# zju3dv/disprcnn

Hardware: AMD Instinct MI355X
Metric: ROI cost-volumes/sec (112x112x48) (higher is better)
Workload: dtype f32 (every convolution of the regressor, the three 32->1 heads included: split-f16 -- each fp32 value carried as hi + lo fp16, 3 f16-MFMA products per fp32 product, f32 accumulate; fp32-class error, tests/test_hip_s16.py.  Head gather and soft-argmin: f32 VALU); 1 GPU; Config A: per ROI pair, features [32,28,28]x2 -> concat cost volume [64,12,28,28] (folded into the first 3D layer's loads, never written) -> 3D stacked-hourglass regressor -> trilinear x4 + softmax + soft-argmin -> disparity [112,112]; maxdisp=48, mindisp=0, parallelism=roi-shard x1 (no collective), weights=closed-form synthetic (disprcnn_amd.utils.synth), BN stats calibrated fixture

## Files before the change

### disprcnn_amd/csrc/s16_cvrows.h

```cpp
#pragma once
#include <hip/hip_runtime.h>
#include <stdint.h>

#include "../../include/disprcnn_hip.h"
#include "s16_ovf.h"

namespace s16cv {

typedef float f32x4 __attribute__((ext_vector_type(4)));
typedef float f32x16 __attribute__((ext_vector_type(16)));
typedef unsigned u32x4 __attribute__((ext_vector_type(4)));
typedef _Float16 f16x8 __attribute__((ext_vector_type(8)));

constexpr int TX = 28;
constexpr int PG = 32;
constexpr int STG_TILE = 8 * 3 * 32 * 16;
constexpr int MAP_B = 32 * 128;
constexpr int MAP_TILE = 9 * MAP_B;
constexpr int STG0 = 0, MAPS0 = 3 * STG_TILE, ZCOL0 = MAPS0 + 3 * MAP_TILE;
constexpr int LDS_BYTES = ZCOL0 + 128;
static_assert(LDS_BYTES <= 160 * 1024, "LDS");

#define S16CV_LDS_PTR(p) ((__attribute__((address_space(3))) void*)(p))
#define S16CV_WAITCNT(vm, lgkm) (((vm) & 15) | (7 << 4) | ((lgkm) << 8) | (((vm) >> 4) << 14))

struct Task { unsigned n; int y, x0, j0, j1; bool valid; };

template <int ROWS>
__device__ __forceinline__ void s16_cvrows_run(const drc_s16conv_params& p, char* lds) {
    const int wave = __builtin_amdgcn_readfirstlane(threadIdx.x >> 6);
    const int lane = threadIdx.x & 63;
    const int xl = lane & 31, hf = lane >> 5;
    const int n_ct = p.cout / 32;
    const int ct = (int)((blockIdx.x >> 3) % n_ct);
    const int D = p.D, H = p.H, W = p.W, lo4 = p.lo4;
    const int Wp = W + 2, Hp = H + 2;
    const long rowB = (long)Wp * 128;
    const long planeB = (long)Hp * rowB;
    const long xcbB = (long)(D + 2) * planeB;
    const long ynB = (long)n_ct * xcbB;
    const long mapnB = planeB;

    const int side = wave >> 1, mlo = (wave & 1) * 4;
    f16x8 wh[5][3][2], wl[5][3][2];
#pragma unroll
    for (int mi = 0; mi < 5; ++mi) {
        const int m = mlo + mi, kd = m / 3, kw = m - kd * 3;
#pragma unroll
        for (int kh = 0; kh < 3; ++kh)
#pragma unroll
            for (int s = 0; s < 2; ++s) {
                const int t = kd * 9 + kh * 3 + kw;
                const char* wb = (const char*)p.w + ((long)(ct * 4 + side * 2 + s) * 54 + t * 2) * 1024 + lane * 16;
                wh[mi][kh][s] = *(const f16x8*)wb;
                wl[mi][kh][s] = *(const f16x8*)(wb + 1024);
            }
    }
    constexpr int PIN_WH = 14;
#pragma unroll
    for (int mi = 0; mi < 5; ++mi)
#pragma unroll
        for (int kh = 0; kh < 3; ++kh)
#pragma unroll
            for (int s = 0; s < 2; ++s) {
                asm volatile("" : "+a"(wl[mi][kh][s]));
                if ((mi * 3 + kh) * 2 + s < PIN_WH) asm volatile("" : "+a"(wh[mi][kh][s]));
            }
    const int q8 = wave * 2 + hf, sg = q8 & 3, jpar = wave >> 1;
    const int grp0 = (sg >> 1) * 4 + (sg & 1), grp1 = grp0 + 2;
    float sc[8], sh[8];
#pragma unroll
    for (int e = 0; e < 8; ++e) {
        const int co = ct * 32 + (sg >> 1) * 16 + (sg & 1) * 4 + 8 * (e >> 2) + (e & 3);
        sc[e] = p.scale[co];
        sh[e] = p.shift[co];
    }
    const float relu_lo = p.relu ? 0.f : -65504.f;
    const unsigned lo_off = (unsigned)(4 * Wp * 16);
    int s_chunk[3], s_row[3], s_col[3];
#pragma unroll
    for (int i = 0; i < 3; ++i) {
        const int idx = (wave * 3 + i) * 64 + lane;
        s_chunk[i] = idx / 96;
        const int rem = idx - s_chunk[i] * 96;
        s_row[i] = rem >> 5;
        s_col[i] = rem & 31;
    }
    if (threadIdx.x < 8) *(f32x4*)(lds + ZCOL0 + threadIdx.x * 16) = (f32x4){0.f, 0.f, 0.f, 0.f};

    const int n_xt = (W + TX - 1) / TX, n_yt = (H + ROWS - 1) / ROWS, n_pg = (D + PG - 1) / PG;
    const unsigned xcd = blockIdx.x & 7, qx = (blockIdx.x >> 3) / n_ct, per_xcd = (gridDim.x >> 3) / n_ct;
    const unsigned items_unit = (unsigned)n_yt * n_xt * n_pg;
    auto task_of = [&](unsigned idx) __attribute__((always_inline)) {
        Task t;
        for (;; ++idx) {
            const unsigned it = idx / ROWS, rr = idx - it * ROWS;
            const unsigned j = it * per_xcd + qx;
            const unsigned nl = j / items_unit;
            unsigned rem = j - nl * items_unit;
            const int yb = (int)(rem / (unsigned)(n_xt * n_pg));
            rem -= (unsigned)yb * (n_xt * n_pg);
            const int xt = (int)(rem / (unsigned)n_pg), pg = (int)(rem - (unsigned)xt * n_pg);
            t.n = nl * 8 + xcd;
            t.valid = t.n < (unsigned)p.N;
            t.y = yb * ROWS + (int)rr;
            t.x0 = xt * TX;
            t.j0 = pg * PG;
            t.j1 = t.j0 + PG < D ? t.j0 + PG : D;
            if (!t.valid || t.y < H) break;
        }
        struct R { Task t; unsigned idx; } r = {t, idx};
        return r;
    };
    struct Reach { int vlo, nb; };
    auto reach_of = [&](const Task& t) __attribute__((always_inline)) {
        Reach r;
        int vlo = t.x0 - (lo4 + t.j1 - 1) - 2, vhi = t.x0 + TX + 1 - (lo4 + t.j0);
        vlo = vlo > 0 ? vlo : 0;
        vhi = vhi < W - 1 ? vhi : W - 1;
        r.vlo = vlo;
        r.nb = vhi >= vlo ? ((vhi - vlo) >> 5) + 1 : 0;
        return r;
    };
    auto stage = [&](const Task& t) __attribute__((always_inline)) {
        const Reach rc = reach_of(t);
        const __amdgpu_buffer_rsrc_t ra = __builtin_amdgcn_make_buffer_rsrc((void*)((const char*)p.left + (long)t.n * mapnB), 0, 0x7FFFFF00, 0x00020000);
        const __amdgpu_buffer_rsrc_t rb = __builtin_amdgcn_make_buffer_rsrc((void*)((const char*)p.right + (long)t.n * mapnB), 0, 0x7FFFFF00, 0x00020000);
#pragma unroll
        for (int T = 0; T < 3; ++T) {
            if (T > rc.nb) break;
            const int v0 = T == 0 ? t.x0 - 1 : rc.vlo + (T - 1) * 32;
#pragma unroll
            for (int i = 0; i < 3; ++i) {
                const int v = v0 + s_col[i];
                const bool ok = v >= -1 && v <= W;
                const unsigned off = ok ? (unsigned)((long)(t.y + s_row[i]) * rowB + (long)s_chunk[i] * (Wp * 16) + (long)(v + 1) * 16) : 0u;
                char* dst = lds + STG0 + T * STG_TILE + (wave * 3 + i) * 1024;
                if (T == 0) __builtin_amdgcn_raw_ptr_buffer_load_lds(ra, S16CV_LDS_PTR(dst), 16, off, 0, 0, 0);
                else __builtin_amdgcn_raw_ptr_buffer_load_lds(rb, S16CV_LDS_PTR(dst), 16, off, 0, 0, 0);
            }
        }
    };
    typedef const __attribute__((address_space(3))) f16x8 lds_frag;
    typedef const __attribute__((address_space(3))) f32x4 lds_f4;
    const __attribute__((address_space(3))) char* ldsl = (const __attribute__((address_space(3))) char*)lds;

    auto cur = task_of(0);
    if (!cur.t.valid) return;
    S16Ovf og;
#pragma unroll
    for (int e = 0; e < 8; ++e) { og.see_raw(sc[e], 3.0e38f); og.see_raw(sh[e], 3.0e38f); }
    stage(cur.t);
#pragma unroll 1
    for (;;) {
        const Task t = cur.t;
        const Reach rc = reach_of(t);
        asm volatile("" ::: "memory");
        __builtin_amdgcn_s_waitcnt(S16CV_WAITCNT(0, 0));
        __builtin_amdgcn_s_barrier();
        asm volatile("" ::: "memory");
        const int nt = side ? rc.nb : 1;
#pragma unroll 1
        for (int T = 0; T < nt; ++T) {
            const int tile = side + T;
            const unsigned fb = (unsigned)(STG0 + tile * STG_TILE + (hf * 96 + xl) * 16);
            f32x16 acc[5];
#pragma unroll
            for (int mi = 0; mi < 5; ++mi)
#pragma unroll
                for (int e = 0; e < 16; ++e) acc[mi][e] = 0.f;
#pragma unroll
            for (int kh = 0; kh < 3; ++kh)
#pragma unroll
                for (int s = 0; s < 2; ++s) {
                    const f16x8 bh = *(lds_frag*)(ldsl + fb + (s * 2 * 96 + kh * 32) * 16);
                    const f16x8 bl = *(lds_frag*)(ldsl + fb + ((4 + s * 2) * 96 + kh * 32) * 16);
#pragma unroll
                    for (int mi = 0; mi < 5; ++mi) acc[mi] = __builtin_amdgcn_mfma_f32_32x32x16_f16(wh[mi][kh][s], bh, acc[mi], 0, 0, 0);
#pragma unroll
                    for (int mi = 0; mi < 5; ++mi) acc[mi] = __builtin_amdgcn_mfma_f32_32x32x16_f16(wh[mi][kh][s], bl, acc[mi], 0, 0, 0);
#pragma unroll
                    for (int mi = 0; mi < 5; ++mi) acc[mi] = __builtin_amdgcn_mfma_f32_32x32x16_f16(wl[mi][kh][s], bh, acc[mi], 0, 0, 0);
                }
#pragma unroll
            for (int mi = 0; mi < 5; ++mi) {
                if (mi == 0 && mlo != 0) continue;
                char* mb = lds + MAPS0 + tile * MAP_TILE + (mlo + mi) * MAP_B + xl * 128;
#pragma unroll
                for (int q = 0; q < 4; ++q)
                    *(f32x4*)(mb + (((2 * q + hf) ^ (xl & 7)) * 16)) = (f32x4){acc[mi][q * 4], acc[mi][q * 4 + 1], acc[mi][q * 4 + 2], acc[mi][q * 4 + 3]};
            }
        }
        asm volatile("" ::: "memory");
        __builtin_amdgcn_s_waitcnt(S16CV_WAITCNT(63, 0));
        __builtin_amdgcn_s_barrier();
        asm volatile("" ::: "memory");
        const auto nxt = task_of(cur.idx + 1);
        if (nxt.t.valid) stage(nxt.t);
        const int x = t.x0 + xl;
        const bool lane_ok = xl < TX && x < W;
        const unsigned long long og_keep = S16Ovf::lanes(lane_ok);
        const __amdgpu_buffer_rsrc_t y16r = __builtin_amdgcn_make_buffer_rsrc((char*)p.y16 + (long)t.n * ynB, 0, 0x7FFFFF00, 0x00020000);
        const unsigned o16 = (unsigned)((long)ct * xcbB + planeB + (long)(t.y + 1) * rowB + (long)sg * (Wp * 16) + (long)(x + 1) * 16);
        const int xa0 = t.x0 - 1;
#pragma unroll 1
        for (int j = t.j0 + jpar; j < t.j1; j += 2) {
            const int u = x - (lo4 + j);
            f32x4 a0 = {0.f, 0.f, 0.f, 0.f}, a1 = {0.f, 0.f, 0.f, 0.f};
#pragma unroll
            for (int kd = 0; kd < 3; ++kd) {
                const bool kd_ok = lane_ok && j + kd - 1 >= 0 && j + kd - 1 < D;
#pragma unroll
                for (int kw = 0; kw < 3; ++kw) {
                    const int cA = x + kw - 1, cB = u + kw - kd;
                    const bool ok = kd_ok && cA >= 0 && cA < W && cB >= 0 && cB < W;
                    const int ia = cA - xa0, ib = cB - rc.vlo;
                    const int m = kd * 3 + kw;
                    const unsigned colA = ok ? (unsigned)(MAPS0 + m * MAP_B + ia * 128) : (unsigned)ZCOL0;
                    const unsigned colB = ok ? (unsigned)(MAPS0 + MAP_TILE + (ib >> 5) * MAP_TILE + m * MAP_B + (ib & 31) * 128) : (unsigned)ZCOL0;
                    const unsigned swA = (unsigned)(ia & 7), swB = (unsigned)(ib & 7);
                    const f32x4 A0 = *(lds_f4*)(ldsl + colA + ((grp0 ^ swA) * 16)), A1 = *(lds_f4*)(ldsl + colA + ((grp1 ^ swA) * 16));
                    const f32x4 B0 = *(lds_f4*)(ldsl + colB + ((grp0 ^ swB) * 16)), B1 = *(lds_f4*)(ldsl + colB + ((grp1 ^ swB) * 16));
                    a0 += A0 + B0;
                    a1 += A1 + B1;
                }
            }
            f16x8 hi, lo;
#pragma unroll
            for (int e = 0; e < 8; ++e) {
                const float s_ = e < 4 ? a0[e & 3] : a1[e & 3];
                float x_ = s_ * sc[e] + sh[e];
                x_ = __builtin_amdgcn_fmed3f(x_, relu_lo, 65504.f);
                og.see(x_, og_keep);
                hi[e] = (_Float16)x_;
                lo[e] = (_Float16)(x_ - (float)hi[e]);
            }
            const unsigned po = lane_ok ? (unsigned)((long)j * planeB) : 0x80000000u;
            __builtin_amdgcn_raw_buffer_store_b128(__builtin_bit_cast(u32x4, hi), y16r, o16 + po, 0, 0);
            __builtin_amdgcn_raw_buffer_store_b128(__builtin_bit_cast(u32x4, lo), y16r, o16 + lo_off + po, 0, 0);
        }
        if (!nxt.t.valid) break;
        cur = nxt;
    }
    og.flush(p.ovf);
}

template <int ROWS>
inline long s16_cvrows_blocks(const drc_s16conv_params& p) {
    const long items = (long)p.N * ((p.H + ROWS - 1) / ROWS) * ((p.W + TX - 1) / TX) * ((p.D + PG - 1) / PG);
    const int n_ct = p.cout / 32;
    long blocks = 256;
    while (blocks > 8 * n_ct && blocks / (2 * n_ct) >= items) blocks /= 2;
    return blocks;
}

}
```

Baseline: 60450 ROI cost-volumes/s.

## Hoist j-invariant A-side map reads out of the disparity loop and rotate B offsets

The A-side map values (left-feature contributions) do not depend on disparity j, so they are now loaded once per task into registers instead of every j iteration. This halves the LDS reads in the inner loop. B-side column offsets are carried in a sliding window of five and shifted by two per step rather than recomputed. The loop also uses a mask-FMA in place of the zero-column trick for A, and adds explicit waitcnt and sched_barrier per kd to interleave reads and adds. The cost is 72 extra VGPRs for the A values, which may lower occupancy, and the forced scheduling may serialise LDS latency.

After: 61440 ROI cost-volumes/s, median of 6. 1.6% higher.

```diff
diff --git a/disprcnn_amd/csrc/s16_cvrows.h b/disprcnn_amd/csrc/s16_cvrows.h
--- a/disprcnn_amd/csrc/s16_cvrows.h
+++ b/disprcnn_amd/csrc/s16_cvrows.h
@@ -20,6 +20,7 @@
 constexpr int STG0 = 0, MAPS0 = 3 * STG_TILE, ZCOL0 = MAPS0 + 3 * MAP_TILE;
 constexpr int LDS_BYTES = ZCOL0 + 128;
 static_assert(LDS_BYTES <= 160 * 1024, "LDS");
+static_assert(ZCOL0 % 64 == 0, "a column's second cout group is its first ^ 32, in the zero column too");
 
 #define S16CV_LDS_PTR(p) ((__attribute__((address_space(3))) void*)(p))
 #define S16CV_WAITCNT(vm, lgkm) (((vm) & 15) | (7 << 4) | ((lgkm) << 8) | (((vm) >> 4) << 14))
@@ -67,7 +68,7 @@
                 if ((mi * 3 + kh) * 2 + s < PIN_WH) asm volatile("" : "+a"(wh[mi][kh][s]));
             }
     const int q8 = wave * 2 + hf, sg = q8 & 3, jpar = wave >> 1;
-    const int grp0 = (sg >> 1) * 4 + (sg & 1), grp1 = grp0 + 2;
+    const int grp0 = (sg >> 1) * 4 + (sg & 1);
     float sc[8], sh[8];
 #pragma unroll
     for (int e = 0; e < 8; ++e) {
@@ -202,28 +203,75 @@
         const unsigned long long og_keep = S16Ovf::lanes(lane_ok);
         const __amdgpu_buffer_rsrc_t y16r = __builtin_amdgcn_make_buffer_rsrc((char*)p.y16 + (long)t.n * ynB, 0, 0x7FFFFF00, 0x00020000);
         const unsigned o16 = (unsigned)((long)ct * xcbB + planeB + (long)(t.y + 1) * rowB + (long)sg * (Wp * 16) + (long)(x + 1) * 16);
-        const int xa0 = t.x0 - 1;
+        auto col_off = [&](unsigned c) __attribute__((always_inline)) { return c * 128u + (((unsigned)grp0 ^ (c & 7u)) << 4); };
+        bool okA[3];
+        f32x4 ar0[9], ar1[9];
+#pragma unroll
+        for (int kw = 0; kw < 3; ++kw) {
+            const int cA = x + kw - 1;
+            okA[kw] = lane_ok && cA >= 0 && cA < W;
+        }
+#pragma unroll
+        for (int m = 0; m < 9; ++m) {
+            const int kw = m % 3;
+            const unsigned oa = okA[kw] ? (unsigned)MAPS0 + col_off((unsigned)(xl + kw) & 31u) : (unsigned)(ZCOL0 - m * MAP_B);
+            ar0[m] = *(lds_f4*)(ldsl + oa + m * MAP_B);
+            ar1[m] = *(lds_f4*)(ldsl + (oa ^ 32u) + m * MAP_B);
+        }
+        auto off_of = [&](int cB) __attribute__((always_inline)) {
+            const int ib = cB - rc.vlo;
+            return (unsigned)(MAPS0 + MAP_TILE) + (unsigned)(ib >> 5) * (unsigned)MAP_TILE + col_off((unsigned)ib & 31u);
+        };
+        unsigned offB[5];
+        bool okB[5];
+        const int jb = t.j0 + jpar;
+#pragma unroll
+        for (int d = 0; d < 5; ++d) {
+            const int cB = x - (lo4 + jb) + d - 2;
+            offB[d] = off_of(cB);
+            okB[d] = (unsigned)cB < (unsigned)W;
+        }
 #pragma unroll 1
-        for (int j = t.j0 + jpar; j < t.j1; j += 2) {
-            const int u = x - (lo4 + j);
+        for (int j = jb; j < t.j1; j += 2) {
             f32x4 a0 = {0.f, 0.f, 0.f, 0.f}, a1 = {0.f, 0.f, 0.f, 0.f};
+            f32x4 B0[9], B1[9];
+            float msk[9];
+            auto read = [&](int kd) __attribute__((always_inline)) {
+                const bool kd_ok = j + kd - 1 >= 0 && j + kd - 1 < D;
+#pragma unroll
+                for (int kw = 0; kw < 3; ++kw) {
+                    const int m = kd * 3 + kw, d = kw - kd + 2;
+                    const bool ok = okA[kw] && kd_ok && okB[d];
+                    const unsigned ob = ok ? offB[d] : (unsigned)(ZCOL0 - m * MAP_B);
+                    B0[m] = *(lds_f4*)(ldsl + ob + m * MAP_B);
+                    B1[m] = *(lds_f4*)(ldsl + (ob ^ 32u) + m * MAP_B);
+                    msk[m] = ok ? 1.f : 0.f;
+                }
+            };
+            auto add = [&](int kd) __attribute__((always_inline)) {
+#pragma unroll
+                for (int kw = 0; kw < 3; ++kw) {
+                    const int m = kd * 3 + kw;
+                    const f32x4 k = {msk[m], msk[m], msk[m], msk[m]};
+                    a0 += __builtin_elementwise_fma(ar0[m], k, B0[m]);
+                    a1 += __builtin_elementwise_fma(ar1[m], k, B1[m]);
+                }
+            };
 #pragma unroll
             for (int kd = 0; kd < 3; ++kd) {
-                const bool kd_ok = lane_ok && j + kd - 1 >= 0 && j + kd - 1 < D;
-#pragma unroll
-                for (int kw = 0; kw < 3; ++kw) {
-                    const int cA = x + kw - 1, cB = u + kw - kd;
-                    const bool ok = kd_ok && cA >= 0 && cA < W && cB >= 0 && cB < W;
-                    const int ia = cA - xa0, ib = cB - rc.vlo;
-                    const int m = kd * 3 + kw;
-                    const unsigned colA = ok ? (unsigned)(MAPS0 + m * MAP_B + ia * 128) : (unsigned)ZCOL0;
-                    const unsigned colB = ok ? (unsigned)(MAPS0 + MAP_TILE + (ib >> 5) * MAP_TILE + m * MAP_B + (ib & 31) * 128) : (unsigned)ZCOL0;
-                    const unsigned swA = (unsigned)(ia & 7), swB = (unsigned)(ib & 7);
-                    const f32x4 A0 = *(lds_f4*)(ldsl + colA + ((grp0 ^ swA) * 16)), A1 = *(lds_f4*)(ldsl + colA + ((grp1 ^ swA) * 16));
-                    const f32x4 B0 = *(lds_f4*)(ldsl + colB + ((grp0 ^ swB) * 16)), B1 = *(lds_f4*)(ldsl + colB + ((grp1 ^ swB) * 16));
-                    a0 += A0 + B0;
-                    a1 += A1 + B1;
-                }
+                read(kd);
+                __builtin_amdgcn_s_waitcnt(S16CV_WAITCNT(63, 0));
+                __builtin_amdgcn_sched_barrier(0);
+                add(kd);
+                __builtin_amdgcn_sched_barrier(0);
+            }
+            offB[4] = offB[2]; offB[3] = offB[1]; offB[2] = offB[0];
+            okB[4] = okB[2]; okB[3] = okB[1]; okB[2] = okB[0];
+#pragma unroll
+            for (int d = 0; d < 2; ++d) {
+                const int cB = x - (lo4 + j + 2) + d - 2;
+                offB[d] = off_of(cB);
+                okB[d] = (unsigned)cB < (unsigned)W;
             }
             f16x8 hi, lo;
 #pragma unroll
```
